# thuml/HashGAN

Hardware: AMD Instinct MI355X
Metric: queries/sec (mAP@R of Q queries vs N-code database, Hamming ranking) (higher is better)
Workload: dtype fp4 (E2M1 0/+-1) x fp4 -> f32 exact distances; u32 xor+popcount elsewhere; f64 AP; 1 GPU; C2: Q=10000 N=1000000 b=64 R=5000 C=10, planted codes; parallelism=1 GPU

## Files before the change

hashgan_amd/csrc/hg_core.hip:

```cpp
#include "hg_ctx.hpp"
#include "hg_host_pack.hpp"

#include <exception>
#include <map>
#include <mutex>
#include <thread>
#include <unistd.h>

thread_local std::string g_err;

int fail(int code, const char* fmt, ...) {
    char buf[512];
    va_list ap;
    va_start(ap, fmt);
    vsnprintf(buf, sizeof buf, fmt, ap);
    va_end(ap);
    g_err = buf;
    return code;
}

const char* const kKernelNames[KI_COUNT] = {"k_hist", "k_hist_reduce", "k_plan", "k_seg_counts", "k_seg_layout", "k_guess",
                                            "k_select", "k_rank_hist", "k_order", "k_rank_fused", "k_match", "k_ap", "k_merge", "k_pack",
                                            "k_real_sample", "k_real_guess", "k_real_select", "k_radix_pass", "k_real_finish", "k_select_mx", "k_rank_cnt", "rccl_allgather", "step_gpu_span", "k_real_rescore",
                                            "k_hist_rel", "k_hist_rel_reduce", "k_graded", "k_grade_hist", "k_grade_hist_reduce", "k_tie_ap"};
// ... 305 lines not shown
                    int64_t idx_base, int64_t n_total) {
    if (!c) return fail(HG_ERR_ARG, "hg_set_database: null context");
    if (N < 1 || !codes || !labels) return fail(HG_ERR_ARG, "hg_set_database: need N >= 1 and data");
    if (b < 1 || b > HG_MAX_BITS) return fail(HG_ERR_ARG, "hg_set_database: b=%d outside 1..%d", b, HG_MAX_BITS);
    if (C < 1) return fail(HG_ERR_ARG, "hg_set_database: C=%d", C);
    if (idx_base < 0 || n_total < N || idx_base + N > n_total || n_total >= 0xFFFFFFFFll)
        return fail(HG_ERR_ARG, "hg_set_database: shard [%lld, %lld) does not fit a database of %lld rows (< 2^32 - 1)",
                    (long long)idx_base, (long long)(idx_base + N), (long long)n_total);
    HG_TRY(c->use());
    c->N = N; c->b = b; c->C = C; c->n_total = n_total;
    c->NW = (b + 31) / 32; c->NB = b + 1; c->LW = (C + 63) / 64;
    c->idx_base = (u32)idx_base;
    c->bpad = 0;
    c->dbf_resident = false;
    HG_TRY(upload_codes(c, c->db, codes, N, (b + 63) / 64, c->NW));
    HG_TRY(c->dblab.reserve((size_t)(N > 0 ? N : 1) * c->LW * 8));
    if (N) HG_HIP(hipMemcpyAsync(c->dblab.p, labels, (size_t)N * c->LW * 8, hipMemcpyHostToDevice, c->stream));
    HG_TRY(c->sync());
    c->stage = ST_DB;
    c->dbx_valid = false;
    c->dbx3_valid = false;
    c->dbx4_valid = false;
    c->dbx8_valid = false;
    c->bet_consecutive_fail = c->shard_bet_fail = 0;
    c->cap_boost = c->real_cap_boost = 1;
    c->crowd_probed = false;
    c->cfg_epoch++;
    c->db_gen++;
    return HG_OK;
}

static int pack_on_device(hg_ctx* c, const float* x, const int64_t* lab, i64 n, DevBuf& codes, DevBuf& labels,
                          DevBuf& feats, int64_t* bad_codes, int64_t* bad_labels, i64 (&census)[3]) {
    const int b = c->b, C = c->C, NW = c->NW, LW = c->LW;
    const int bpad = (b + 15) / 16 * 16;
    c->bpad = bpad;
    const size_t fb = (size_t)n * bpad * 4, lb = (size_t)n * C * 8;
    HG_TRY(feats.reserve(fb + 256));
    HG_TRY(c->stage_in.reserve(lb));
    HG_TRY(c->badcnt.reserve(32));
    HG_TRY(codes.reserve((size_t)n * NW * 4 + 64 * 4));
    HG_TRY(labels.reserve((size_t)n * LW * 8));
    HG_HIP(hipMemsetAsync(c->badcnt.p, 0, 32, c->stream));
    if (bpad != b) HG_HIP(hipMemsetAsync(feats.p, 0, fb, c->stream));
    HG_HIP(hipMemcpy2DAsync(feats.p, (size_t)bpad * 4, x, (size_t)b * 4, (size_t)b * 4, (size_t)n, hipMemcpyHostToDevice, c->stream));
    c->t_begin(KI_PACK);
// ... 153 lines not shown
    if (N < 1 || !host_x || !host_labels) return fail(HG_ERR_ARG, "hg_set_database_f32: need N >= 1 and data");
    if (b < 1 || b > HG_MAX_BITS) return fail(HG_ERR_ARG, "hg_set_database_f32: b=%d outside 1..%d", b, HG_MAX_BITS);
    if (C < 1) return fail(HG_ERR_ARG, "hg_set_database_f32: C=%d", C);
    if (idx_base < 0 || n_total < N || idx_base + N > n_total || n_total >= 0xFFFFFFFFll)
        return fail(HG_ERR_ARG, "hg_set_database_f32: shard [%lld, %lld) does not fit a database of %lld rows (< 2^32 - 1)",
                    (long long)idx_base, (long long)(idx_base + N), (long long)n_total);
    HG_TRY(c->use());
    c->N = N; c->b = b; c->C = C; c->n_total = n_total;
    c->NW = (b + 31) / 32; c->NB = b + 1; c->LW = (C + 63) / 64;
    c->idx_base = (u32)idx_base;
    if (c->opt.host_pack) {
        HG_TRY(pack_on_host(c, host_x, host_labels, N, c->db, c->dblab, c->dbf, (int)c->opt.keep_floats, &c->dbf_resident,
                            bad_codes, bad_labels, c->census_db));
    } else {
        HG_TRY(pack_on_device(c, host_x, host_labels, N, c->db, c->dblab, c->dbf, bad_codes, bad_labels, c->census_db));
        c->dbf_resident = true;
    }
    if (!c->dbf_resident) c->bpad = 0;
    c->stage = ST_DB;
    c->dbx_valid = false;
    c->dbx3_valid = false;
    c->dbx4_valid = false;
    c->dbx8_valid = false;
    c->dbfx_valid = false;
    c->dbfb_valid = false;
    c->bet_consecutive_fail = c->shard_bet_fail = 0;
    c->cap_boost = c->real_cap_boost = 1;
    c->crowd_probed = false;
    c->cfg_epoch++;
    c->db_gen++;
    return HG_OK;
}

static __global__ __launch_bounds__(256) void k_copy_in(const u32* __restrict__ src_a, u32* __restrict__ dst_a, const i64 na, const int sw, const int dw,
                                                        const u32* __restrict__ src_b, u32* __restrict__ dst_b, const i64 nb) {
    const i64 i = (i64)blockIdx.x * 256 + threadIdx.x;
    if (i < na) { const i64 r = i / dw; dst_a[i] = src_a[r * sw + (i - r * dw)]; }
    else if (i - na < nb) dst_b[i - na] = src_b[i - na];
}

static void queries_replaced(hg_ctx* c, i64 old_q, bool had_q) {
    const bool carry = had_q && old_q == c->Q && c->map_warm_R >= 0 && c->map_warm_cfg == c->cfg_epoch;
    c->cfg_epoch++;
    c->q_gen++;
    if (carry) c->map_warm_cfg = c->cfg_epoch;
}

int hg_set_queries_f32(hg_ctx* c, const float* host_x, const int64_t* host_labels, int64_t Q, int64_t* bad_codes,
                       int64_t* bad_labels) {
    HG_TRY(need(c, ST_DB, "hg_set_queries_f32", "hg_set_database"));
    if (Q < 1 || !host_x || !host_labels) return fail(HG_ERR_ARG, "hg_set_queries_f32: need Q >= 1 and data");
    if (Q > 0x7FFFFFC0ll) return fail(HG_ERR_ARG, "hg_set_queries_f32: Q too large");
    const i64 old_q = c->Q;
    const bool had_q = (c->stage & ST_Q) != 0;
    c->Q = Q;
    if (c->opt.host_pack) {
        const int saved_bpad = c->bpad;
        HG_TRY(pack_on_host(c, host_x, host_labels, Q, c->qc, c->qlab, c->qf, c->dbf_resident ? 1 : 0, &c->qf_resident,
                            bad_codes, bad_labels, c->census_q));
        if (!c->qf_resident) c->bpad = saved_bpad;
    } else {
        HG_TRY(pack_on_device(c, host_x, host_labels, Q, c->qc, c->qlab, c->qf, bad_codes, bad_labels, c->census_q));
        c->qf_resident = true;
    }
    c->stage = ST_DB | ST_Q;
    c->qx_valid = false;
    queries_replaced(c, old_q, had_q);
    return HG_OK;
}

int hg_get_packed(hg_ctx* c, int which, uint32_t* host_codes, uint64_t* host_labels) {
    HG_TRY(need(c, which ? (ST_DB | ST_Q) : ST_DB, "hg_get_packed", "hg_set_database / hg_set_queries"));
    const i64 n = which ? c->Q : c->N;
    DevBuf& cd = which ? c->qc : c->db;
    DevBuf& lb = which ? c->qlab : c->dblab;
    if (host_codes) HG_HIP(hipMemcpyAsync(host_codes, cd.p, (size_t)n * c->NW * 4, hipMemcpyDeviceToHost, c->stream));
    if (host_labels) HG_HIP(hipMemcpyAsync(host_labels, lb.p, (size_t)n * c->LW * 8, hipMemcpyDeviceToHost, c->stream));
    return c->sync();
}

int hg_set_queries(hg_ctx* c, const uint64_t* codes, const uint64_t* labels, int64_t Q) {
    HG_TRY(need(c, ST_DB, "hg_set_queries", "hg_set_database"));
    if (Q < 1 || !codes || !labels) return fail(HG_ERR_ARG, "hg_set_queries: need Q >= 1 and data");
    if (Q > 0x7FFFFFC0ll) return fail(HG_ERR_ARG, "hg_set_queries: Q too large");
    const i64 old_q = c->Q;
    const bool had_q = (c->stage & ST_Q) != 0;
    c->Q = Q;
    const int W = (c->b + 63) / 64;
    const size_t cb = (size_t)Q * W * 8, lb = (size_t)Q * c->LW * 8;
// ... 3 lines not shown
    if (qs.cap < cb + lb) {
        pin_free(qs.pin, qs.cap);
        qs.pin = nullptr; qs.cap = 0;
        HG_HIP(pin_alloc(&qs.pin, cb + lb, &qs.cap));
    }
    if (!qs.ev) HG_HIP(hipEventCreateWithFlags(&qs.ev, hipEventDisableTiming));
    memcpy(qs.pin, codes, cb);
    memcpy((char*)qs.pin + cb, labels, lb);
    HG_TRY(c->qc.reserve((size_t)Q * c->NW * 4 + 64 * 4));
    HG_TRY(c->qlab.reserve(lb));
    if (cb + lb <= ((size_t)4 << 20)) {
        const i64 nc = (i64)Q * c->NW, nl = (i64)Q * c->LW * 2;
        hipLaunchKernelGGL(k_copy_in, dim3(grid_for(nc + nl)), dim3(256), 0, c->stream, (const u32*)qs.pin, c->qc.as<u32>(), nc, 2 * W, c->NW,
                           (const u32*)((const char*)qs.pin + cb), c->qlab.as<u32>(), nl);
        HG_TRY(c->check_launch("k_copy_in"));
    } else {
        HG_TRY(upload_codes(c, c->qc, (const uint64_t*)qs.pin, Q, W, c->NW));
        HG_HIP(hipMemcpyAsync(c->qlab.p, (const char*)qs.pin + cb, lb, hipMemcpyHostToDevice, c->stream));
    }
    HG_HIP(hipEventRecord(qs.ev, c->stream));
    qs.used = true;
    c->stage = ST_DB | ST_Q;
    c->qx_valid = false;
    c->qf_resident = false;
    queries_replaced(c, old_q, had_q);
    return HG_OK;
}

extern "C++" int do_match(hg_ctx* c) {
    const Geo& g = c->geo;
    const i64 nKB = (g.R + 255) / 256;
    const i64 blocks = nKB * g.Q;
    if (blocks > 0x7FFFFFFFll) return fail(HG_ERR_ARG, "hg_match: Q*R too large for one launch");
    c->t_begin(KI_MATCH);
    hipLaunchKernelGGL(k_match, dim3((unsigned)blocks), dim3(256), 0, c->stream, c->out_idx.as<u32>(),
                       c->dblab.as<u64>(), c->qlab.as<u64>(), c->mbits.as<u64>(), c->RW, (int)nKB, g);
    c->t_end();
    HG_TRY(c->check_launch("k_match"));
    c->stage |= ST_MATCH;
    c->stage &= ~(unsigned)ST_AP;
    return HG_OK;
}

int hg_match(hg_ctx* c) {
    HG_TRY(need(c, ST_SELECT, "hg_match", "hg_select"));
    if (c->stage & ST_MATCH) return HG_OK;
// ... 264 lines not shown
        c->own_stream = true;
    }
    if (c->sub) c->sub->stream = c->stream;
    return HG_OK;
}

namespace {
struct OptionKey { const char* key; i64 Options::*field; bool flag; i64 lo, hi; const char* range; };
constexpr i64 kMax = INT64_MAX;
constexpr OptionKey flag(const char* k, i64 Options::*f) { return {k, f, true, 0, 1, nullptr}; }
constexpr OptionKey ranged(const char* k, i64 Options::*f, i64 lo, i64 hi, const char* range) { return {k, f, false, lo, hi, range}; }
const OptionKey kOptionKeys[] = {
    ranged("target_units", &Options::target_units, 1, kMax, "target_units must be >= 1"),
    ranged("min_segment", &Options::min_segment, 16, kMax, "min_segment must be >= 16"),
    ranged("max_segments", &Options::max_segments, 1, kMax, "max_segments must be >= 1"),
    ranged("sample_stride", &Options::sample_stride, 0, 1024, "sample_stride must be 0 (auto) .. 1024"),
    ranged("guess_sigma", &Options::guess_sigma, 0, 64, "guess_sigma must be 0..64"),
    ranged("cand_budget_x10", &Options::cand_budget_x10, 11, 1000, "cand_budget_x10 must be 11..1000"),
    flag("second_bet", &Options::second_bet),
    flag("crowd_probe", &Options::crowd_probe),
    flag("select_mfma", &Options::select_mfma),
    ranged("select_packed", &Options::select_packed, INT64_MIN, kMax, nullptr),
    flag("compact_records", &Options::compact_records),
    ranged("hist_mfma", &Options::hist_mfma, 0, 2, "hist_mfma must be 0, 1 or 2"),
    ranged("rank_lds", &Options::rank_lds, 0, 2, "rank_lds must be 0, 1 or 2"),
    ranged("rank_slices", &Options::rank_slices, 0, kMax, "rank_slices must be >= 0 (the smallest R it takes; 0: off)"),
    ranged("rank_dense", &Options::rank_dense, 0, 2, "rank_dense must be 0 or 1 (2 is accepted and means 1)"),
    ranged("rank_dense_gbm", &Options::rank_dense_gbm, -1, 1, "rank_dense_gbm must be -1, 0 or 1"),
    ranged("dense_budget_mb", &Options::dense_budget_mb, 1, kMax, "dense_budget_mb must be >= 1"),
    flag("all_rows_shortcut", &Options::all_rows_shortcut),
    flag("fuse_ap", &Options::fuse_ap),
    flag("inline_leftovers", &Options::inline_leftovers),
    flag("ap_wide", &Options::ap_wide),
    flag("ap_recip", &Options::ap_recip),
#if HG_PROBES
    ranged("probe_select", &Options::probe_select, INT64_MIN, kMax, nullptr),
#endif
    flag("stage_sync", &Options::stage_sync),
    flag("defer_verdict", &Options::defer_verdict),
    flag("staged_lists", &Options::staged_lists),
    flag("step_graph", &Options::step_graph),
    ranged("step_streams", &Options::step_streams, 1, 2, "step_streams must be 1 or 2"),
    ranged("timing_every", &Options::timing_every, 1, 1024, "timing_every must be 1..1024"),
    flag("host_pack", &Options::host_pack),
    ranged("keep_floats", &Options::keep_floats, 0, 2, "keep_floats must be 0, 1 or 2"),
    ranged("real_mfma", &Options::real_mfma, 0, 2, "real_mfma must be 0, 1 or 2"),
// ... 101 lines not shown
        const char* rest = key + 5;
        int kind = -1;
        if (!strncmp(rest, "us_", 3)) { kind = 0; rest += 3; }
        else if (!strncmp(rest, "n_", 2)) { kind = 1; rest += 2; }
        else if (!strncmp(rest, "max_us_", 7)) { kind = 2; rest += 7; }
        int ph = -1;
        for (int i = 0; i < HP_COUNT; ++i) if (!strcmp(rest, kHostPhaseNames[i])) ph = i;
        if (kind < 0 || ph < 0) return fail(HG_ERR_ARG, "hg_get_stat: unknown key '%s'", key);
        *value = kind == 0 ? g_host_ns[ph].load() / 1000 : kind == 1 ? g_host_calls[ph].load() : g_host_max_ns[ph].load() / 1000;
    }
    else if (!strcmp(key, "graph_replays")) *value = c->graph_replays;
    else if (!strcmp(key, "cut_beyond_planes")) {
        u32 v = 0;
        if (c->beyond.p) {
            HG_HIP(hipMemcpyAsync(&v, c->beyond.p, 4, hipMemcpyDeviceToHost, c->stream));
            HG_TRY(c->sync());
        }
        *value = v;
    }
    else if (!strcmp(key, "map_async_steps")) *value = c->map_async_steps;
    else if (!strcmp(key, "map_async_redone")) *value = c->map_async_redone;
    else if (!strcmp(key, "map_overlapped_steps")) *value = c->map_overlapped;
    else if (!strcmp(key, "segments")) *value = c->geo.S;
    else if (!strcmp(key, "records_kept")) {
        const Geo& g = c->geo;
        *value = -1;
        if (c->optimistic && c->sl_cnt.p && c->sl_cnt.cap >= (size_t)g.S * g.Qpad * 4) {
            HG_TRY(c->use());
            HG_TRY(c->sync());
            std::vector<u32> h((size_t)g.S * g.Qpad);
            HG_HIP(hipMemcpy(h.data(), c->sl_cnt.p, h.size() * 4, hipMemcpyDeviceToHost));
            i64 total = 0;
            for (int s = 0; s < g.S; ++s) for (int q = 0; q < g.Q; ++q) total += h[(size_t)s * g.Qpad + q];
            *value = total;
        }
    }
    else return fail(HG_ERR_ARG, "hg_get_stat: unknown key '%s'", key);
    return HG_OK;
}

int hg_get_census(hg_ctx* c, int queries, int64_t out[4]) {
    if (!c || !out) return fail(HG_ERR_ARG, "hg_get_census: null argument");
    const i64* cs = queries ? c->census_q : c->census_db;
    out[0] = cs[0]; out[1] = cs[1]; out[2] = cs[2];
    out[3] = (queries ? c->qf_resident : c->dbf_resident) ? 1 : 0;
    return HG_OK;
// ... 37 lines not shown
```

hashgan_amd/csrc/hg_ctx.hpp:

```cpp
#pragma once
#include "hg_kernels.hpp"
#pragma GCC visibility push(default)
#include "../../include/hashgan_amd.h"
#pragma GCC visibility pop

#include <rccl/rccl.h>
#include <atomic>
#include <chrono>
#include <cmath>
#include <cstdarg>
#include <cstdio>
#include <cstdlib>
#include <cstring>
#include <string>
#include <utility>
#include <vector>

using namespace hg;

extern thread_local std::string g_err;
int fail(int code, const char* fmt, ...);

#define HG_HIP(expr)                                                                         \
    do {                                                                                     \
// ... 150 lines not shown
                KI_ORDER, KI_RANK_FUSED, KI_MATCH, KI_AP, KI_MERGE, KI_PACK, KI_REAL_SAMPLE, KI_REAL_GUESS, KI_REAL_SELECT,
                KI_RADIX, KI_REAL_FINISH, KI_SELECT_MX, KI_RANK_LDS, KI_COMM, KI_STEP, KI_REAL_RESCORE, KI_HIST_REL, KI_HIST_REL_REDUCE,
                KI_GRADED, KI_GRADE_HIST, KI_GRADE_HIST_REDUCE, KI_TIE_AP, KI_COUNT };
enum Stage { ST_NONE = 0, ST_DB = 1, ST_Q = 2, ST_HIST = 4, ST_PLAN = 8, ST_SELECT = 16, ST_MATCH = 32, ST_AP = 64 };
extern const char* const kKernelNames[KI_COUNT];

void build_shape(int n, ApShape& sh);

struct Pending { int id; hipEvent_t a, b; };

struct Options {
    i64 target_units = 16384;
    i64 min_segment = 256;
    i64 max_segments = 2048;
    i64 optimistic = 1;
    i64 sample_stride = 0;
    i64 guess_sigma = 5;
    i64 cand_budget_x10 = 40;
    i64 second_bet = 1;
    i64 crowd_probe = 1;
    i64 select_mfma = 1;
    i64 select_packed = 3;
    i64 compact_records = 1;
    i64 hist_mfma = 2;
    i64 rank_lds = 2;
    i64 rank_slices = 7000;
    i64 rank_dense = 1;
    i64 rank_dense_gbm = -1;
    i64 dense_budget_mb = 16384;
    i64 all_rows_shortcut = 1;
    i64 fuse_ap = 1;
    i64 inline_leftovers = 1;
    i64 ap_wide = 1;
    i64 ap_recip = 1;
    i64 probe_select = 0;
    i64 stage_sync = 1;
    i64 defer_verdict = 0;
    i64 staged_lists = 1;
    i64 step_graph = 0;
    i64 step_streams = 2;
    i64 timing_every = 1;
    i64 host_pack = 1;
    i64 keep_floats = 2;
    i64 real_mfma = 2;
    i64 real_sample_half = 1;
    i64 real_second_sample = 1;
// ... 74 lines not shown
    Options opt;

    i64 N = 0, Q = 0, R = 0, n_total = 0;
    int b = 0, C = 0, NW = 0, NB = 0, LW = 0;
    u32 idx_base = 0;
    int G = 1, rank = 0;

    bool crowd_probed = false;
    i64 crowd_x100 = 0;
    i64 cap_boost = 1;
    i64 real_cap_boost = 1;
    bool leftovers_expected = false;
    bool last_leftovers_inline = false;

    bool want_lists = true;
    i64 bet_runs = 0, bet_fallbacks = 0, bet_requeried = 0;
    i64 rank_leftovers = 0;
    int bet_consecutive_fail = 0;
    int shard_bet_fail = 0;
    hg_ctx* sub = nullptr;
    bool is_sub = false;

    bool dbx_valid = false, qx_valid = false, dbx8_valid = false, dbx3_valid = false, dbx4_valid = false;
    bool hist_pairs = false;
    i64 bet_rebets = 0;
    bool rh_done = false;
    unsigned long long rh_q_gen = 0, rh_db_gen = 0;
    i64 rh_Q = 0, rh_Qpad = 0, rh_NB = 0;
    int last_rel_hist = 0;
    bool gr_done = false, gr_kept = false;
    unsigned long long gr_q_gen = 0, gr_db_gen = 0;
    i64 gr_Q = 0, gr_R = 0;
    int gr_nk = 0;
    bool gh_done = false;
    unsigned long long gh_q_gen = 0, gh_db_gen = 0;
    i64 gh_Q = 0, gh_Qpad = 0, gh_G = 0;
    bool ta_done = false;
    unsigned long long ta_q_gen = 0, ta_db_gen = 0;
    i64 ta_Q = 0;
    int ta_nR = 0;
    bool verdict_pending = false, verdict_known = false;
    int verdict_flag = 0;
    void* pin = nullptr;
    size_t pin_cap = 0;
    struct MapSlot {
        void* pin = nullptr; size_t cap = 0; hipEvent_t ev = nullptr;
// ... 29 lines not shown
    i64 real_requeried = 0;
    int bpad = 0;
    i64 census_db[3] = {0, 0, 0}, census_q[3] = {0, 0, 0};
    hipStream_t stream2 = nullptr;
    hipEvent_t stream2_ev = nullptr;
    size_t fstage_cap = 0;
    void* fstage = nullptr;
    hipEvent_t fstage_ev[4] = {nullptr, nullptr, nullptr, nullptr};
    void* hpk = nullptr;
    size_t hpk_cap = 0;
    bool dbf_resident = false, qf_resident = false;
    RealState real;
    bool real_lists = false;
    i64 shapes_for_R = -1;
    i64 recip_for_R = -1;

    ncclComm_t comm = nullptr;
    int comm_rank = 0, comm_world = 1;

    DevBuf db, dblab, qc, qlab;
    DevBuf dbf, qf;
    DevBuf dbx, qx;
    DevBuf dbx8;
    DevBuf rh_part, rh_all, rh_rel;
    DevBuf gr_tab, gr_out, gr_grades;
    DevBuf gh_part, gh_tab;
    DevBuf ta_tab, ta_out;
    DevBuf dbx3;
    DevBuf dbx4;
    DevBuf dbfx;
    DevBuf dbfb, xmax2;
    DevBuf shapes, ap_recip;
    DevBuf seglt, segtie;
    DevBuf mbits2;
    DevBuf part;
    DevBuf obuf[2];
    DevBuf beyond;
    DevBuf stage_in, badcnt;
    DevBuf flist;
    DevBuf dbytes;
    DevBuf samp, thr, sortA, sortB, scores, gtab;
    DevBuf sampx;
    DevBuf cntq;
    DevBuf krows;
    DevBuf thr2;
    DevBuf hist2;
    DevBuf gathered[4], scratch[4], comm_tmp, gath_idx, gath_dist;

    template <class F> void for_each_buf(F&& f) {
        for (DevBuf* d : {&db, &dblab, &qc, &qlab, &dbf, &qf}) f(*d, BUF_TABLE);
        for (DevBuf* d : {&dbx, &qx, &dbx8, &dbx3, &dbx4, &dbfx, &dbfb, &xmax2, &shapes, &ap_recip}) f(*d, BUF_DERIVED);
        for (DevBuf* d : {&seglt, &segtie, &mbits2, &part, &obuf[0], &obuf[1], &beyond, &stage_in, &badcnt, &flist, &dbytes, &samp, &thr,
                          &sortA, &sortB, &scores, &gtab, &sampx, &cntq, &krows, &thr2, &hist2, &comm_tmp, &gath_idx, &gath_dist, &rh_part, &rh_all, &rh_rel,
                          &gr_tab, &gr_out, &gr_grades, &gh_part, &gh_tab, &ta_tab, &ta_out})
            f(*d, BUF_WORK);
        for (DevBuf& d : gathered) f(d, BUF_WORK);
        for (DevBuf& d : scratch) f(d, BUF_WORK);
        for_each_step_buf(f);
        ws_b.for_each_step_buf(f);
    }
    void forget_derived() {
        dbx_valid = qx_valid = dbx8_valid = dbx3_valid = dbx4_valid = dbfx_valid = dbfb_valid = false;
        rh_done = false;
        gr_done = gr_kept = gh_done = ta_done = false;
        shapes_for_R = recip_for_R = -1;
        outblk_q = ws_b.outblk_q = -1;
    }

    struct StepGraph {
        hipGraph_t graph = nullptr;
        hipGraphExec_t exec = nullptr;
        unsigned long long epoch = 0, cfg = 0, seen_epoch = 0, seen_cfg = 0;
        i64 R = -1, seen_R = -1;
        int timing = -1, seen_timing = -1;
        StepState left;
        std::vector<Pending> evs;
    } sg;
    unsigned long long cfg_epoch = 1;
    bool capturing = false;
    i64 graph_replays = 0, graph_captures = 0;

    int timing = 0;
    double t_ms[KI_COUNT] = {0};
    i64 t_n[KI_COUNT] = {0};
    std::vector<Pending> pending;
// ... 89 lines not shown
inline int grid_for(i64 n, int per_block = 256) { return (int)((n + per_block - 1) / per_block); }
inline int padded_grid(int nBlk) { return (nBlk + 7) / 8 * 8; }

int need(hg_ctx* c, unsigned st, const char* who, const char* what);
int upload_codes(hg_ctx* c, DevBuf& dst, const uint64_t* host, i64 n, int W, int NW);
int ensure_pin(hg_ctx* c, size_t need_b);
int do_match(hg_ctx* c);
int ensure_ap_tables(hg_ctx* c, bool* use_recip);
int do_ap_range(hg_ctx* c, i64 q0, i64 nq, const u32* only = nullptr);
inline int do_ap(hg_ctx* c) { return do_ap_range(c, 0, c->geo.Q); }
int ensure_out_block(hg_ctx* c);
int read_plan_flag(hg_ctx* c, int* flag);
int launch_min_topr(hg_ctx* c, const u32* idx_all, const u8* dist_all, i64 n, int G);
hg_ctx* requery_child(hg_ctx* c, i64 nF);
int stage_ap_download(hg_ctx* c, void* dst = nullptr);
int wait_verdict(hg_ctx* c, bool staged, int* flag);
void make_geometry(hg_ctx* c);
Geo hist_geometry(const hg_ctx* c);
int set_R(hg_ctx* c, int64_t R, int G, int rank);
int launch_hist(hg_ctx* c);
int launch_hist_rel(hg_ctx* c, const Geo& g);
int launch_select_valu(hg_ctx* c, int lw, bool optimistic);
int launch_select_dense(hg_ctx* c, int lw);
int ensure_mx_images(hg_ctx* c, bool need_db);
int launch_hist_mx(hg_ctx* c);
int launch_select_mx(hg_ctx* c, int lw, const int* cut);
int launch_select_mx3(hg_ctx* c, int lw, const int* cut);
int launch_select_mx4(hg_ctx* c, int lw, const int* cut);
int preload_valu(); int preload_mx(); int preload_mx1(); int preload_real(); int preload_seq();
void comm_release(hg_ctx* c);

#define HG_DISPATCH_NW(fn, c, ...)                              \
    switch ((c)->NW) {                                          \
        case 1: return fn<1>(c, ##__VA_ARGS__);                 \
        case 2: return fn<2>(c, ##__VA_ARGS__);                 \
        case 3: return fn<3>(c, ##__VA_ARGS__);                 \
        case 4: return fn<4>(c, ##__VA_ARGS__);                 \
        case 5: return fn<5>(c, ##__VA_ARGS__);                 \
        case 6: return fn<6>(c, ##__VA_ARGS__);                 \
        case 7: return fn<7>(c, ##__VA_ARGS__);                 \
        case 8: return fn<8>(c, ##__VA_ARGS__);                 \
        default: return fail(HG_ERR_ARG, "unsupported code length: %d words", (c)->NW); \
    }
```

hashgan_amd/csrc/hg_hist_i8.hpp:

```cpp
#pragma once
#include "hg_kernels.hpp"
#include "hg_hist_mx.hpp"

namespace hg {

typedef int i32x16 __attribute__((ext_vector_type(16)));
typedef __attribute__((address_space(3))) u32 lds_u32;

__device__ __forceinline__ void lds_add_at(const u32 addr, const u32 inc) {
#if defined(__HIP_DEVICE_COMPILE__)
    __hip_atomic_fetch_add((lds_u32*)addr, inc, __ATOMIC_RELAXED, __HIP_MEMORY_SCOPE_WORKGROUP);
#else
    (void)addr; (void)inc;
#endif
}

__device__ __forceinline__ uint4 bits16_to_bytes(const u32 bits, const u32 one, const u32 zero) {
    u32 w[4];
#pragma unroll
    for (int d = 0; d < 4; ++d) {
        u32 v = 0;
#pragma unroll
        for (int i = 0; i < 4; ++i) v |= (((bits >> (4 * d + i)) & 1u) ? one : zero) << (8 * i);
        w[d] = v;
    }
    return uint4{w[0], w[1], w[2], w[3]};
}

static __global__ __launch_bounds__(256) void k_expand_db_i8(const u32* __restrict__ db, uint4* __restrict__ img, i64 N, i64 n16, int NW) {
    const i64 i = (i64)blockIdx.x * 256 + threadIdx.x;
    if (i >= n16 * NW * 2) return;
    const i64 row = i / (NW * 2);
    const int c = (int)(i - row * NW * 2), m = c >> 1, hh = c & 1;
    const u32 word = row < N ? db[row * NW + m] : 0u;
    img[(((row >> 4) * NW + m) * 2 + hh) * 16 + (row & 15)] = bits16_to_bytes((word >> (16 * hh)) & 0xFFFFu, 8u, 0u);
}

constexpr int hist_i8_cols(bool pack16) { return pack16 ? 1 : 2; }

template <int NW, bool PACK16>
__global__ __launch_bounds__(256) __attribute__((amdgpu_waves_per_eu(4, 4)))
void k_hist_i8(const u32* __restrict__ qc, const u8* __restrict__ dbx8, u32* __restrict__ hist, const Geo g) {
    extern __shared__ __attribute__((aligned(16))) u32 hlds[];
    constexpr int QT = 2, WQ = 32 * QT;
    const int lb = logical_block(g.nBlk);
    if (lb < 0) return;
    const int lane = threadIdx.x & 63;
    const int wave = __builtin_amdgcn_readfirstlane(threadIdx.x >> 6);
    const int nQB = g.nQT;
    const int sp = lb / nQB, qb = lb - sp * nQB;
    const int h = lane >> 5, j = lane & 31;
    const int NB = g.NB, b = g.NB - 1;
    const i64 lo0 = (i64)(2 * sp) * g.L, lo1 = lo0 + g.L;
    const i64 len0 = (lo0 + g.L < g.N ? g.L : g.N - lo0);
    const i64 len1 = lo1 >= g.N ? 0 : (lo1 + g.L < g.N ? g.L : g.N - lo1);
    const i64 mylen = h ? len1 : len0;
    const i64 ntile = ((len0 > len1 ? len0 : len1) + 15) / 16;
    const i64 NG = (g.N + 15) >> 4;
    const int stride = g.hist_stride;

    constexpr int NCOL = hist_i8_cols(PACK16);
    u32* col = hlds + wave * NCOL * NB * 32;
    for (int i = lane; i < NCOL * NB * 32; i += 64) col[i] = 0u;

    const int q0w = (qb * WPB + wave) * WQ;
    i32x4 bq[QT][NW];
    i32x16 biasv[QT];
    u32 inc[QT];
#pragma unroll
    for (int t = 0; t < QT; ++t) {
        const int q = q0w + t * 32 + j;
        int pop = 0;
#pragma unroll
        for (int m = 0; m < NW; ++m) {
            const u32 word = q < g.Q ? qc[(i64)q * NW + m] : 0u;
            pop += __builtin_popcount(word);
            const int first = 32 * m + 16 * h;
            const u32 valid = b - first >= 16 ? 0xFFFFu : (b - first <= 0 ? 0u : (1u << (b - first)) - 1u);
            const u32 bits = (word >> (16 * h)) & 0xFFFFu;
            const uint4 neg = bits16_to_bytes(bits & valid, 0xF0u, 0u);
            const uint4 pos = bits16_to_bytes(~bits & valid, 0x10u, 0u);
            bq[t][m] = i32x4{(int)(neg.x | pos.x), (int)(neg.y | pos.y), (int)(neg.z | pos.z), (int)(neg.w | pos.w)};
        }
        u32* c0 = col + (PACK16 ? 0 : t * NB * 32) + j;
        const int base = (int)(u32)(size_t)(lds_u32*)c0 + 128 * pop;
#pragma unroll
        for (int r = 0; r < 16; ++r) biasv[t][r] = base;
        inc[t] = PACK16 ? (t ? 65536u : 1u) : 1u;
    }
    wave_lds_sync();

    const int ah = (j >> 2) & 1;
    const int ar = (j & 3) + 4 * (j >> 3);
    const i64 ag0 = (ah ? lo1 : lo0) >> 4;
    auto chunk = [&](const i64 T, const int m) -> i32x4 {
        i64 G = ag0 + T;
        G = G < NG ? G : NG - 1;
        return *(const i32x4*)(dbx8 + ((((G * NW + m) * 2 + h) * 16 + ar) * 16));
    };
    i32x4 av[NW];
    if (ntile > 0) {
#pragma unroll
        for (int m = 0; m < NW; ++m) av[m] = chunk(0, m);
    }
    for (i64 T = 0; T < ntile; T += stride) {
        i32x4 an[NW];
        const i64 Tn = T + stride < ntile ? T + stride : T;
#pragma unroll
        for (int m = 0; m < NW; ++m) an[m] = chunk(Tn, m);
        const i64 left = mylen - T * 16;
        const bool whole = __all(left >= 16);
#pragma unroll
        for (int t = 0; t < QT; ++t) {
            i32x16 acc = biasv[t];
#pragma unroll
            for (int m = 0; m < NW; ++m) acc = __builtin_amdgcn_mfma_i32_32x32x32_i8(av[m], bq[t][m], acc, 0, 0, 0);
            if (whole) {
#pragma unroll
                for (int r = 0; r < 16; ++r)
                    lds_add_at((u32)acc[r], inc[t]);
            } else {
#pragma unroll
                for (int r = 0; r < 16; ++r)
                    if ((i64)r < left) lds_add_at((u32)acc[r], inc[t]);
            }
        }
#pragma unroll
        for (int m = 0; m < NW; ++m) av[m] = an[m];
    }
    wave_lds_sync();
    const int q = q0w + lane;
    if (q < g.Qpad) {
        u32* __restrict__ out = hist + (i64)sp * NB * g.Qpad + q;
        const int dn = g.hcap > 0 && g.hcap < NB ? g.hcap : NB;
        for (int d = 0; d < dn; ++d) {
            const u32 v = PACK16 ? (col[d * 32 + j] >> (16 * h)) & 0xFFFFu : col[(h * NB + d) * 32 + j];
            out[(i64)d * g.Qpad] = v;
        }
    }
}

}
```

hashgan_amd/csrc/hg_pairs_mx.hip:

```cpp
#include "hg_ctx.hpp"
#include "hg_mx_drain.hpp"
#include "hg_select_mx.hpp"
#include "hg_select_mx3.hpp"
#include "hg_select_mx4.hpp"
#include "hg_hist_mx.hpp"
#include "hg_hist_i8.hpp"

int ensure_mx_images(hg_ctx* c, const bool need_db) {
    const int NW = c->NW, NM = (NW + 1) / 2;
    if (need_db && !c->dbx_valid) {
        const i64 n16 = (c->N + 15) / 16 * 16;
        HG_TRY(c->dbx.reserve((size_t)(n16 > 0 ? n16 : 16) * NM * 32));
        const i64 items = n16 * 2 * NM;
        c->t_begin(KI_PACK);
        if (items) hipLaunchKernelGGL(k_expand_db, dim3(grid_for(items)), dim3(256), 0, c->stream, c->db.as<u32>(),
                                      c->dbx.as<uint4>(), (i64)c->N, n16, NW, NM);
        c->t_end();
        HG_TRY(c->check_launch("k_expand_db"));
        c->dbx_valid = true;
    }
    if (!c->qx_valid) {
        const i64 qpad = ((i64)c->Q + 511) / 512 * 512;
        HG_TRY(c->qx.reserve((size_t)qpad * NM * 32));
        const i64 items = qpad * 2 * NM;
        c->t_begin(KI_PACK);
        hipLaunchKernelGGL(k_expand_queries, dim3(grid_for(items)), dim3(256), 0, c->stream, c->qc.as<u32>(), c->qx.as<uint4>(),
                           (i64)c->Q, qpad, NW, NM);
        c->t_end();
        HG_TRY(c->check_launch("k_expand_queries"));
        c->qx_valid = true;
    }
    return HG_OK;
}


namespace {
template <int NW> int launch_hist_mx_t(hg_ctx* c) {
    HG_TRY(ensure_mx_images(c, true));
    Geo g = c->geo;
    const int nSP = (g.S + 1) / 2;
    const int nQB = (g.Q + 255) / 256;
    g.nQT = nQB;
    g.nUnits = (i64)nSP * nQB;
    g.wpb = WPB;
    g.nBlk = (int)g.nUnits;
    const i64 tiles_per_half = ((g.L + 15) / 16 + g.hist_stride - 1) / g.hist_stride;
    const i64 visited_per_pair = 2 * tiles_per_half * 16;
    const bool pack16 = visited_per_pair < 65536;
    const size_t lds = (size_t)WPB * (pack16 ? 1 : 2) * g.NB * 32 * 4;
    c->t_begin(KI_HIST);
    if (pack16) {
        hipLaunchKernelGGL((k_hist_mx<NW, true>), dim3(padded_grid(g.nBlk)), dim3(256), lds, c->stream, c->qc.as<u32>(), c->qx.as<u8>(),
                           c->dbx.as<u8>(), c->hist.as<u32>(), g);
// ... 27 lines not shown
    g.nQT = nQB;
    g.nUnits = (i64)nSP * nQB;
    g.wpb = P::WPB;
    g.nBlk = (int)g.nUnits;
    const PackedLds L = packed_lds_layout<P>(NW, LW);
    if (L.total > 64 * 1024)
        HG_HIP(hipFuncSetAttribute(reinterpret_cast<const void*>(kernel), hipFuncAttributeMaxDynamicSharedMemorySize, L.total));
    SelArgs a{cut, c->sl_start.as<u32>(), c->sl_tie.as<u32>(), c->sl_cnt.as<u32>(),
              c->failq.as<u32>(), c->cap, c->crow, 1, c->sstar.as<int>(), (int)c->opt.probe_select};
    c->t_begin(KI_SELECT_MX);
    hipLaunchKernelGGL(kernel, dim3(padded_grid(g.nBlk)), dim3(64 * P::WPB), (size_t)L.total, c->stream, c->qc.as<u32>(),
                       c->qlab.as<u64>(), c->qx.as<u8>(), c->db.as<u32>(), image.as<u8>(), c->dblab.as<u64>(), a,
                       c->cand.as<u8>(), g);
    c->t_end();
    return c->check_launch(kernel_name);
}
template <int NW, int LW> int launch_select_mx3_t(hg_ctx* c, const int* cut) {
    return launch_select_packed<M3Pack>(c, cut, NW, LW, c->dbx3, c->dbx3_valid, k_expand_db3, "k_expand_db3", &k_select_mx3<NW, LW>, "k_select_mx3");
}
template <int NW, int LW> int launch_select_mx4_t(hg_ctx* c, const int* cut) {
    return launch_select_packed<M4Pack>(c, cut, NW, LW, c->dbx4, c->dbx4_valid, k_expand_db4, "k_expand_db4", &k_select_mx4<NW, LW>, "k_select_mx4");
}

template <int NW> int launch_hist_i8_t(hg_ctx* c) {
    if (!c->dbx8_valid) {
        const i64 n16 = (c->N + 15) / 16 * 16;
        HG_TRY(c->dbx8.reserve((size_t)n16 * NW * 32));
        c->t_begin(KI_PACK);
        hipLaunchKernelGGL(k_expand_db_i8, dim3(grid_for(n16 * NW * 2)), dim3(256), 0, c->stream, c->db.as<u32>(), c->dbx8.as<uint4>(),
                           (i64)c->N, n16, NW);
        c->t_end();
        HG_TRY(c->check_launch("k_expand_db_i8"));
        c->dbx8_valid = true;
    }
    Geo g = c->geo;
    const int nSP = (g.S + 1) / 2;
    const int nQB = (g.Q + 255) / 256;
    g.nQT = nQB;
    g.nUnits = (i64)nSP * nQB;
    g.wpb = WPB;
    g.nBlk = (int)g.nUnits;
    const i64 tiles_per_half = ((g.L + 15) / 16 + g.hist_stride - 1) / g.hist_stride;
    const bool pack16 = 2 * tiles_per_half * 16 < 65536;
    const size_t lds = (size_t)WPB * hist_i8_cols(pack16) * g.NB * 32 * 4;
    c->t_begin(KI_HIST);
    if (pack16) {
        if (lds > 64 * 1024)
            HG_HIP(hipFuncSetAttribute(reinterpret_cast<const void*>(&k_hist_i8<NW, true>), hipFuncAttributeMaxDynamicSharedMemorySize, (int)lds));
        hipLaunchKernelGGL((k_hist_i8<NW, true>), dim3(padded_grid(g.nBlk)), dim3(256), lds, c->stream, c->qc.as<u32>(), c->dbx8.as<u8>(),
                           c->hist.as<u32>(), g);
    } else {
        if (lds > 64 * 1024)
            HG_HIP(hipFuncSetAttribute(reinterpret_cast<const void*>(&k_hist_i8<NW, false>), hipFuncAttributeMaxDynamicSharedMemorySize, (int)lds));
        hipLaunchKernelGGL((k_hist_i8<NW, false>), dim3(padded_grid(g.nBlk)), dim3(256), lds, c->stream, c->qc.as<u32>(), c->dbx8.as<u8>(),
                           c->hist.as<u32>(), g);
    }
    c->t_end();
    return c->check_launch("k_hist_i8");
}
}

int launch_hist_mx(hg_ctx* c) {
    if (c->opt.hist_mfma == 2 && c->NW <= 4) {
        switch (c->NW) {
            case 1: return launch_hist_i8_t<1>(c);
            case 2: return launch_hist_i8_t<2>(c);
            case 3: return launch_hist_i8_t<3>(c);
            default: return launch_hist_i8_t<4>(c);
        }
    }
    HG_DISPATCH_NW(launch_hist_mx_t, c)
}


int launch_select_mx4(hg_ctx* c, int lw, const int* cut) {
    if (c->NW < 3 || c->NW > 4 || lw < 1 || lw > 2) return fail(HG_ERR_ARG, "k_select_mx4 takes codes of 65..128 bits and 1..128 classes");
    if (c->NW == 3) return lw == 1 ? launch_select_mx4_t<3, 1>(c, cut) : launch_select_mx4_t<3, 2>(c, cut);
    return lw == 1 ? launch_select_mx4_t<4, 1>(c, cut) : launch_select_mx4_t<4, 2>(c, cut);
}

int launch_select_mx3(hg_ctx* c, int lw, const int* cut) {
// ... 11 lines not shown
```

hashgan_amd/csrc/hg_seq.hip:

```cpp
#include "hg_ctx.hpp"
#include <chrono>
#include "hg_select_mx.hpp"
#include "hg_select_mx3.hpp"
#include "hg_select_mx4.hpp"
#include "hg_hist_mx.hpp"
#include "hg_hist_rel.hpp"
#include "hg_graded.hpp"
#include "hg_tie_ap.hpp"
#include "hg_rank_cnt.hpp"
#include "hg_rank_lean.hpp"
#include "hg_rank_dense.hpp"

constexpr i64 SAMPLE_RATIO = 2;

void make_geometry(hg_ctx* c) {
    Geo& g = c->geo;
    g.Q = (int)c->Q;
    g.nQT = (int)((c->Q + 63) / 64);
    g.Qpad = g.nQT * 64;
    g.NW = c->NW; g.NB = c->NB; g.LW = c->LW;
    g.N = c->N; g.R = c->R; g.idx_base = c->idx_base;
    i64 S = (c->opt.target_units + g.nQT - 1) / g.nQT;
    if (S > c->opt.max_segments) S = c->opt.max_segments;
    const i64 maxS = (c->N + c->opt.min_segment - 1) / c->opt.min_segment;
// ... 1482 lines not shown

int hg_topr(hg_ctx* c, int64_t R) {
    HG_TRY(need(c, ST_DB | ST_Q, "hg_topr", "hg_set_database + hg_set_queries"));
    return run_oneshot(c, R, true, false);
}

int hg_map(hg_ctx* c, int64_t R, double* host_ap, int64_t* host_rel) {
    HG_TRY(need(c, ST_DB | ST_Q, "hg_map", "hg_set_database + hg_set_queries"));
    const i64 fails0 = c->bet_fallbacks + c->bet_requeried + c->bet_rebets, left0 = c->rank_leftovers;
    c->last_leftovers_inline = false;
    HG_TRY(run_oneshot(c, R, false, true));
    HG_TRY(hg_get_ap(c, host_ap, host_rel));
    if (c->optimistic && c->bet_fallbacks + c->bet_requeried + c->bet_rebets == fails0 && (c->rank_leftovers == left0 || c->last_leftovers_inline) && !c->is_sub) {
        c->map_warm_cfg = c->cfg_epoch; c->map_warm_epoch = g_alloc_epoch; c->map_warm_R = R;
        if (c->opt.step_streams >= 2 && c->own_stream && !c->stream_b) HG_TRY(stream_create(c->device, &c->stream_b));
    } else {
        c->map_warm_R = -1;
    }
    return HG_OK;
}

static int prepare_shared(hg_ctx* c, int64_t R, bool* enqueued) {
    *enqueued = false;
    if (c->opt.select_mfma && !c->qx_valid) { HG_TRY(ensure_mx_images(c, false)); *enqueued = true; }
    const bool recip = c->opt.ap_recip && R <= (1ll << 20);
    if (c->shapes_for_R != R || (recip && c->recip_for_R != R)) {
        HG_TRY(set_R(c, R, 1, 0));
        bool use_recip = false;
        HG_TRY(ensure_ap_tables(c, &use_recip));
        *enqueued = true;
    }
    return HG_OK;
}

static int enqueue_bet_on_b(hg_ctx* c, hg_ctx::MapSlot& m, int64_t R, int stride, bool tail_fork) {
    if (!c->stream_b) HG_TRY(stream_create(c->device, &c->stream_b));
    if (!c->ev_pre) HG_HIP(hipEventCreateWithFlags(&c->ev_pre, hipEventDisableTiming));
    if (!c->ev_fork) HG_HIP(hipEventCreateWithFlags(&c->ev_fork, hipEventDisableTiming));
    if (tail_fork || !c->pre_valid) {
        HG_HIP(hipEventRecord(c->ev_fork, c->stream));
        HG_HIP(hipStreamWaitEvent(c->stream_b, c->ev_fork, 0));
    } else {
        HG_HIP(hipStreamWaitEvent(c->stream_b, c->ev_pre, 0));
    }
    c->b_open = false;
    const unsigned long long e0 = g_alloc_epoch.load();
    c->swap_step();
// ... 105 lines not shown
```

Baseline: 12.53 million queries/s.

## Precompute int8 query images and run hist kernel as persistent blocks

Adds a separate kernel that expands query codes into int8 MFMA operand images plus popcounts once and caches them, so the histogram kernel loads them instead of rebuilding them per block. The histogram kernel becomes persistent: the grid is sized from occupancy times CU count, and each block walks a contiguous run of (query block, segment) units. It reloads query operands only when the query block changes and drains LDS counters with atomic exchange so they can be reused. This cuts the per-block query expansion and launch cost, in exchange for an extra image buffer, an extra pre-pass kernel and serial per-block work that may balance less evenly.

```diff
diff --git a/hashgan_amd/csrc/hg_core.hip b/hashgan_amd/csrc/hg_core.hip
--- a/hashgan_amd/csrc/hg_core.hip
+++ b/hashgan_amd/csrc/hg_core.hip
@@ -351,6 +351,7 @@
     c->dbx3_valid = false;
     c->dbx4_valid = false;
     c->dbx8_valid = false;
+    c->qx8_valid = false;
     c->bet_consecutive_fail = c->shard_bet_fail = 0;
     c->cap_boost = c->real_cap_boost = 1;
     c->crowd_probed = false;
@@ -550,6 +551,7 @@
     c->dbx3_valid = false;
     c->dbx4_valid = false;
     c->dbx8_valid = false;
+    c->qx8_valid = false;
     c->dbfx_valid = false;
     c->dbfb_valid = false;
     c->bet_consecutive_fail = c->shard_bet_fail = 0;
@@ -593,6 +595,7 @@
     }
     c->stage = ST_DB | ST_Q;
     c->qx_valid = false;
+    c->qx8_valid = false;
     queries_replaced(c, old_q, had_q);
     return HG_OK;
 }
@@ -642,6 +645,7 @@
     qs.used = true;
     c->stage = ST_DB | ST_Q;
     c->qx_valid = false;
+    c->qx8_valid = false;
     c->qf_resident = false;
     queries_replaced(c, old_q, had_q);
     return HG_OK;
@@ -952,6 +956,7 @@
     flag("select_mfma", &Options::select_mfma),
     ranged("select_packed", &Options::select_packed, INT64_MIN, kMax, nullptr),
     flag("compact_records", &Options::compact_records),
+    ranged("hist_blocks", &Options::hist_blocks, 0, 1 << 20, "hist_blocks must be 0 (auto) .. 1048576"),
     ranged("hist_mfma", &Options::hist_mfma, 0, 2, "hist_mfma must be 0, 1 or 2"),
     ranged("rank_lds", &Options::rank_lds, 0, 2, "rank_lds must be 0, 1 or 2"),
     ranged("rank_slices", &Options::rank_slices, 0, kMax, "rank_slices must be >= 0 (the smallest R it takes; 0: off)"),
@@ -1099,6 +1104,9 @@
     else if (!strcmp(key, "map_async_redone")) *value = c->map_async_redone;
     else if (!strcmp(key, "map_overlapped_steps")) *value = c->map_overlapped;
     else if (!strcmp(key, "segments")) *value = c->geo.S;
+    else if (!strcmp(key, "segment_rows")) *value = c->geo.L;
+    else if (!strcmp(key, "hist_stride")) *value = c->geo.hist_stride;
+    else if (!strcmp(key, "hist_blocks_used")) *value = c->hist_blocks_used;
     else if (!strcmp(key, "records_kept")) {
         const Geo& g = c->geo;
         *value = -1;
diff --git a/hashgan_amd/csrc/hg_ctx.hpp b/hashgan_amd/csrc/hg_ctx.hpp
--- a/hashgan_amd/csrc/hg_ctx.hpp
+++ b/hashgan_amd/csrc/hg_ctx.hpp
@@ -196,6 +196,7 @@
     i64 select_mfma = 1;
     i64 select_packed = 3;
     i64 compact_records = 1;
+    i64 hist_blocks = 0;
     i64 hist_mfma = 2;
     i64 rank_lds = 2;
     i64 rank_slices = 7000;
@@ -316,6 +317,10 @@
     bool is_sub = false;
 
     bool dbx_valid = false, qx_valid = false, dbx8_valid = false, dbx3_valid = false, dbx4_valid = false;
+    bool qx8_valid = false;
+    i64 hist_occ_key = -1;
+    int hist_occ = 0;
+    i64 hist_blocks_used = 0;
     bool hist_pairs = false;
     i64 bet_rebets = 0;
     bool rh_done = false;
@@ -391,6 +396,7 @@
     DevBuf dbf, qf;
     DevBuf dbx, qx;
     DevBuf dbx8;
+    DevBuf qx8;
     DevBuf rh_part, rh_all, rh_rel;
     DevBuf gr_tab, gr_out, gr_grades;
     DevBuf gh_part, gh_tab;
@@ -418,7 +424,7 @@
 
     template <class F> void for_each_buf(F&& f) {
         for (DevBuf* d : {&db, &dblab, &qc, &qlab, &dbf, &qf}) f(*d, BUF_TABLE);
-        for (DevBuf* d : {&dbx, &qx, &dbx8, &dbx3, &dbx4, &dbfx, &dbfb, &xmax2, &shapes, &ap_recip}) f(*d, BUF_DERIVED);
+        for (DevBuf* d : {&dbx, &qx, &dbx8, &qx8, &dbx3, &dbx4, &dbfx, &dbfb, &xmax2, &shapes, &ap_recip}) f(*d, BUF_DERIVED);
         for (DevBuf* d : {&seglt, &segtie, &mbits2, &part, &obuf[0], &obuf[1], &beyond, &stage_in, &badcnt, &flist, &dbytes, &samp, &thr,
                           &sortA, &sortB, &scores, &gtab, &sampx, &cntq, &krows, &thr2, &hist2, &comm_tmp, &gath_idx, &gath_dist, &rh_part, &rh_all, &rh_rel,
                           &gr_tab, &gr_out, &gr_grades, &gh_part, &gh_tab, &ta_tab, &ta_out})
@@ -429,7 +435,7 @@
         ws_b.for_each_step_buf(f);
     }
     void forget_derived() {
-        dbx_valid = qx_valid = dbx8_valid = dbx3_valid = dbx4_valid = dbfx_valid = dbfb_valid = false;
+        dbx_valid = qx_valid = qx8_valid = dbx8_valid = dbx3_valid = dbx4_valid = dbfx_valid = dbfb_valid = false;
         rh_done = false;
         gr_done = gr_kept = gh_done = ta_done = false;
         shapes_for_R = recip_for_R = -1;
@@ -565,7 +571,7 @@
 int launch_hist_rel(hg_ctx* c, const Geo& g);
 int launch_select_valu(hg_ctx* c, int lw, bool optimistic);
 int launch_select_dense(hg_ctx* c, int lw);
-int ensure_mx_images(hg_ctx* c, bool need_db);
+int ensure_mx_images(hg_ctx* c, bool need_db, bool need_q8 = false);
 int launch_hist_mx(hg_ctx* c);
 int launch_select_mx(hg_ctx* c, int lw, const int* cut);
 int launch_select_mx3(hg_ctx* c, int lw, const int* cut);
diff --git a/hashgan_amd/csrc/hg_hist_i8.hpp b/hashgan_amd/csrc/hg_hist_i8.hpp
--- a/hashgan_amd/csrc/hg_hist_i8.hpp
+++ b/hashgan_amd/csrc/hg_hist_i8.hpp
@@ -36,107 +36,141 @@
     img[(((row >> 4) * NW + m) * 2 + hh) * 16 + (row & 15)] = bits16_to_bytes((word >> (16 * hh)) & 0xFFFFu, 8u, 0u);
 }
 
+static __global__ __launch_bounds__(256) void k_expand_queries_i8(const u32* __restrict__ qc, uint4* __restrict__ img, int* __restrict__ pop,
+                                                                  i64 Q, i64 qpad, int NW, int b) {
+    const i64 i = (i64)blockIdx.x * 256 + threadIdx.x;
+    if (i >= qpad * NW * 2) return;
+    const int lane = (int)(i & 63), h = lane >> 5, j = lane & 31;
+    const i64 c = i >> 6, tile = c / NW;
+    const int m = (int)(c - tile * NW);
+    const i64 q = tile * 32 + j;
+    const u32 word = q < Q ? qc[q * NW + m] : 0u;
+    const int first = 32 * m + 16 * h;
+    const u32 valid = b - first >= 16 ? 0xFFFFu : (b - first <= 0 ? 0u : (1u << (b - first)) - 1u);
+    const u32 bits = (word >> (16 * h)) & 0xFFFFu;
+    const uint4 neg = bits16_to_bytes(bits & valid, 0xF0u, 0u);
+    const uint4 pos = bits16_to_bytes(~bits & valid, 0x10u, 0u);
+    img[i] = uint4{neg.x | pos.x, neg.y | pos.y, neg.z | pos.z, neg.w | pos.w};
+    if (m == 0 && h == 0) {
+        int p = 0;
+        for (int w = 0; w < NW; ++w) p += __builtin_popcount(q < Q ? qc[q * NW + w] : 0u);
+        pop[q] = p;
+    }
+}
+inline size_t hist_i8_qimage_bytes(i64 qpad, int NW) { return (size_t)qpad * NW * 32; }
+
 constexpr int hist_i8_cols(bool pack16) { return pack16 ? 1 : 2; }
 
 template <int NW, bool PACK16>
 __global__ __launch_bounds__(256) __attribute__((amdgpu_waves_per_eu(4, 4)))
-void k_hist_i8(const u32* __restrict__ qc, const u8* __restrict__ dbx8, u32* __restrict__ hist, const Geo g) {
+void k_hist_i8(const u8* __restrict__ qx8, const int* __restrict__ qpop, const u8* __restrict__ dbx8, u32* __restrict__ hist, const Geo g,
+               const int nSP, const int run, const int rem) {
     extern __shared__ __attribute__((aligned(16))) u32 hlds[];
     constexpr int QT = 2, WQ = 32 * QT;
     const int lb = logical_block(g.nBlk);
     if (lb < 0) return;
     const int lane = threadIdx.x & 63;
     const int wave = __builtin_amdgcn_readfirstlane(threadIdx.x >> 6);
-    const int nQB = g.nQT;
-    const int sp = lb / nQB, qb = lb - sp * nQB;
     const int h = lane >> 5, j = lane & 31;
-    const int NB = g.NB, b = g.NB - 1;
-    const i64 lo0 = (i64)(2 * sp) * g.L, lo1 = lo0 + g.L;
-    const i64 len0 = (lo0 + g.L < g.N ? g.L : g.N - lo0);
-    const i64 len1 = lo1 >= g.N ? 0 : (lo1 + g.L < g.N ? g.L : g.N - lo1);
-    const i64 mylen = h ? len1 : len0;
-    const i64 ntile = ((len0 > len1 ? len0 : len1) + 15) / 16;
+    const int NB = g.NB;
     const i64 NG = (g.N + 15) >> 4;
     const int stride = g.hist_stride;
+    const int dn = g.hcap > 0 && g.hcap < NB ? g.hcap : NB;
+    const int u0 = lb * run + (lb < rem ? lb : rem), nu = run + (lb < rem ? 1 : 0);
+    int qb = u0 / nSP, sp = u0 - qb * nSP;
 
     constexpr int NCOL = hist_i8_cols(PACK16);
     u32* col = hlds + wave * NCOL * NB * 32;
     for (int i = lane; i < NCOL * NB * 32; i += 64) col[i] = 0u;
-
-    const int q0w = (qb * WPB + wave) * WQ;
-    i32x4 bq[QT][NW];
-    i32x16 biasv[QT];
-    u32 inc[QT];
-#pragma unroll
-    for (int t = 0; t < QT; ++t) {
-        const int q = q0w + t * 32 + j;
-        int pop = 0;
-#pragma unroll
-        for (int m = 0; m < NW; ++m) {
-            const u32 word = q < g.Q ? qc[(i64)q * NW + m] : 0u;
-            pop += __builtin_popcount(word);
-            const int first = 32 * m + 16 * h;
-            const u32 valid = b - first >= 16 ? 0xFFFFu : (b - first <= 0 ? 0u : (1u << (b - first)) - 1u);
-            const u32 bits = (word >> (16 * h)) & 0xFFFFu;
-            const uint4 neg = bits16_to_bytes(bits & valid, 0xF0u, 0u);
-            const uint4 pos = bits16_to_bytes(~bits & valid, 0x10u, 0u);
-            bq[t][m] = i32x4{(int)(neg.x | pos.x), (int)(neg.y | pos.y), (int)(neg.z | pos.z), (int)(neg.w | pos.w)};
-        }
-        u32* c0 = col + (PACK16 ? 0 : t * NB * 32) + j;
-        const int base = (int)(u32)(size_t)(lds_u32*)c0 + 128 * pop;
-#pragma unroll
-        for (int r = 0; r < 16; ++r) biasv[t][r] = base;
-        inc[t] = PACK16 ? (t ? 65536u : 1u) : 1u;
-    }
     wave_lds_sync();
 
     const int ah = (j >> 2) & 1;
     const int ar = (j & 3) + 4 * (j >> 3);
-    const i64 ag0 = (ah ? lo1 : lo0) >> 4;
-    auto chunk = [&](const i64 T, const int m) -> i32x4 {
-        i64 G = ag0 + T;
-        G = G < NG ? G : NG - 1;
-        return *(const i32x4*)(dbx8 + ((((G * NW + m) * 2 + h) * 16 + ar) * 16));
-    };
-    i32x4 av[NW];
-    if (ntile > 0) {
+    i32x4 bq[QT][NW];
+    int base[QT] = {0, 0};
+    int cur = -1;
+    for (int u = 0; u < nu; ++u) {
+        const int q0w = (qb * WPB + wave) * WQ;
+        if (q0w < g.Qpad) {
+            if (qb != cur) {
+                cur = qb;
 #pragma unroll
-        for (int m = 0; m < NW; ++m) av[m] = chunk(0, m);
-    }
-    for (i64 T = 0; T < ntile; T += stride) {
-        i32x4 an[NW];
-        const i64 Tn = T + stride < ntile ? T + stride : T;
+                for (int t = 0; t < QT; ++t) {
+                    const i64 tile = (i64)(q0w >> 5) + t;
 #pragma unroll
-        for (int m = 0; m < NW; ++m) an[m] = chunk(Tn, m);
-        const i64 left = mylen - T * 16;
-        const bool whole = __all(left >= 16);
+                    for (int m = 0; m < NW; ++m) bq[t][m] = *(const i32x4*)(qx8 + ((tile * NW + m) * 64 + lane) * 16);
+                    u32* c0 = col + (PACK16 ? 0 : t * NB * 32) + j;
+                    base[t] = (int)(u32)(size_t)(lds_u32*)c0 + 128 * qpop[q0w + t * 32 + j];
+                }
+            }
+            i32x16 biasv[QT];
 #pragma unroll
-        for (int t = 0; t < QT; ++t) {
-            i32x16 acc = biasv[t];
+            for (int t = 0; t < QT; ++t)
 #pragma unroll
-            for (int m = 0; m < NW; ++m) acc = __builtin_amdgcn_mfma_i32_32x32x32_i8(av[m], bq[t][m], acc, 0, 0, 0);
-            if (whole) {
+                for (int r = 0; r < 16; ++r) biasv[t][r] = base[t];
+            const i64 lo0 = (i64)(2 * sp) * g.L, lo1 = lo0 + g.L;
+            const i64 len0 = (lo0 + g.L < g.N ? g.L : g.N - lo0);
+            const i64 len1 = lo1 >= g.N ? 0 : (lo1 + g.L < g.N ? g.L : g.N - lo1);
+            const i64 mylen = h ? len1 : len0;
+            const i64 ntile = ((len0 > len1 ? len0 : len1) + 15) / 16;
+            const i64 ag0 = (ah ? lo1 : lo0) >> 4;
+            auto chunk = [&](const i64 T, const int m) -> i32x4 {
+                i64 G = ag0 + T;
+                G = G < NG ? G : NG - 1;
+                return *(const i32x4*)(dbx8 + ((((G * NW + m) * 2 + h) * 16 + ar) * 16));
+            };
+            i32x4 av[NW];
 #pragma unroll
-                for (int r = 0; r < 16; ++r)
-                    lds_add_at((u32)acc[r], inc[t]);
+            for (int m = 0; m < NW; ++m) av[m] = chunk(0, m);
+            for (i64 T = 0; T < ntile; T += stride) {
+                i32x4 an[NW];
+                const i64 Tn = T + stride < ntile ? T + stride : T;
+#pragma unroll
+                for (int m = 0; m < NW; ++m) an[m] = chunk(Tn, m);
+                const i64 left = mylen - T * 16;
+                const bool whole = __all(left >= 16);
+#pragma unroll
+                for (int t = 0; t < QT; ++t) {
+                    i32x16 acc = biasv[t];
+#pragma unroll
+                    for (int m = 0; m < NW; ++m) acc = __builtin_amdgcn_mfma_i32_32x32x32_i8(av[m], bq[t][m], acc, 0, 0, 0);
+                    const u32 inc = PACK16 && t ? 65536u : 1u;
+                    if (whole) {
+#pragma unroll
+                        for (int r = 0; r < 16; ++r)
+                            lds_add_at((u32)acc[r], inc);
+                    } else {
+#pragma unroll
+                        for (int r = 0; r < 16; ++r)
+                            if ((i64)r < left) lds_add_at((u32)acc[r], inc);
+                    }
+                }
+#pragma unroll
+                for (int m = 0; m < NW; ++m) av[m] = an[m];
+            }
+            wave_lds_sync();
+            int ol = lane;
+            __asm__ volatile("" : "+v"(ol));
+            const int oh = ol >> 5, oj = ol & 31;
+            if (PACK16) {
+                u32* __restrict__ out = hist + ((i64)sp * NB + oh) * g.Qpad + q0w + oj;
+                u32* c = col + ol;
+                for (int d = oh; d < dn; d += 2, c += 64, out += 2 * (i64)g.Qpad) {
+                    const u32 v = __hip_atomic_exchange(c, 0u, __ATOMIC_RELAXED, __HIP_MEMORY_SCOPE_WORKGROUP);
+                    out[0] = v & 0xFFFFu;
+                    out[32] = v >> 16;
+                }
             } else {
-#pragma unroll
-                for (int r = 0; r < 16; ++r)
-                    if ((i64)r < left) lds_add_at((u32)acc[r], inc[t]);
+                u32* __restrict__ out = hist + (i64)sp * NB * g.Qpad + q0w + ol;
+                u32* c = col + oh * NB * 32 + oj;
+                for (int d = 0; d < dn; ++d, c += 32, out += g.Qpad) {
+                    const u32 v = __hip_atomic_exchange(c, 0u, __ATOMIC_RELAXED, __HIP_MEMORY_SCOPE_WORKGROUP);
+                    out[0] = v;
+                }
             }
+            wave_lds_sync();
         }
-#pragma unroll
-        for (int m = 0; m < NW; ++m) av[m] = an[m];
-    }
-    wave_lds_sync();
-    const int q = q0w + lane;
-    if (q < g.Qpad) {
-        u32* __restrict__ out = hist + (i64)sp * NB * g.Qpad + q;
-        const int dn = g.hcap > 0 && g.hcap < NB ? g.hcap : NB;
-        for (int d = 0; d < dn; ++d) {
-            const u32 v = PACK16 ? (col[d * 32 + j] >> (16 * h)) & 0xFFFFu : col[(h * NB + d) * 32 + j];
-            out[(i64)d * g.Qpad] = v;
-        }
+        if (++sp == nSP) { sp = 0; ++qb; }
     }
 }
 
diff --git a/hashgan_amd/csrc/hg_pairs_mx.hip b/hashgan_amd/csrc/hg_pairs_mx.hip
--- a/hashgan_amd/csrc/hg_pairs_mx.hip
+++ b/hashgan_amd/csrc/hg_pairs_mx.hip
@@ -6,7 +6,7 @@
 #include "hg_hist_mx.hpp"
 #include "hg_hist_i8.hpp"
 
-int ensure_mx_images(hg_ctx* c, const bool need_db) {
+int ensure_mx_images(hg_ctx* c, const bool need_db, const bool need_q8) {
     const int NW = c->NW, NM = (NW + 1) / 2;
     if (need_db && !c->dbx_valid) {
         const i64 n16 = (c->N + 15) / 16 * 16;
@@ -29,6 +29,17 @@
         c->t_end();
         HG_TRY(c->check_launch("k_expand_queries"));
         c->qx_valid = true;
+    }
+    if (need_q8 && !c->qx8_valid) {
+        const i64 qpad = ((i64)c->Q + 255) / 256 * 256;
+        const size_t img = hist_i8_qimage_bytes(qpad, NW);
+        HG_TRY(c->qx8.reserve(img + (size_t)qpad * 4));
+        c->t_begin(KI_PACK);
+        hipLaunchKernelGGL(k_expand_queries_i8, dim3(grid_for(qpad * NW * 2)), dim3(256), 0, c->stream, c->qc.as<u32>(), c->qx8.as<uint4>(),
+                           (int*)(c->qx8.as<char>() + img), (i64)c->Q, qpad, NW, c->b);
+        c->t_end();
+        HG_TRY(c->check_launch("k_expand_queries_i8"));
+        c->qx8_valid = true;
     }
     return HG_OK;
 }
@@ -102,7 +113,29 @@
     return launch_select_packed<M4Pack>(c, cut, NW, LW, c->dbx4, c->dbx4_valid, k_expand_db4, "k_expand_db4", &k_select_mx4<NW, LW>, "k_select_mx4");
 }
 
+template <int NW, bool PACK16> int launch_hist_i8_p(hg_ctx* c, Geo g, const int nSP, const size_t lds) {
+    const void* fn = reinterpret_cast<const void*>(&k_hist_i8<NW, PACK16>);
+    if (lds > 64 * 1024) HG_HIP(hipFuncSetAttribute(fn, hipFuncAttributeMaxDynamicSharedMemorySize, (int)lds));
+    const i64 key = ((i64)lds << 4) | (NW << 1) | (PACK16 ? 1 : 0);
+    if (c->hist_occ_key != key) {
+        int per_cu = 0;
+        HG_HIP(hipOccupancyMaxActiveBlocksPerMultiprocessor(&per_cu, fn, 256, lds));
+        c->hist_occ = per_cu > 0 ? per_cu : 1;
+        c->hist_occ_key = key;
+    }
+    const i64 want = c->opt.hist_blocks > 0 ? c->opt.hist_blocks : (i64)c->n_cu * c->hist_occ;
+    g.nBlk = (int)(want < g.nUnits ? want : g.nUnits);
+    c->hist_blocks_used = g.nBlk;
+    const size_t img = hist_i8_qimage_bytes(((i64)c->Q + 255) / 256 * 256, NW);
+    c->t_begin(KI_HIST);
+    hipLaunchKernelGGL((k_hist_i8<NW, PACK16>), dim3(padded_grid(g.nBlk)), dim3(256), lds, c->stream, c->qx8.as<u8>(),
+                       (const int*)(c->qx8.as<char>() + img), c->dbx8.as<u8>(), c->hist.as<u32>(), g, nSP,
+                       (int)(g.nUnits / g.nBlk), (int)(g.nUnits % g.nBlk));
+    c->t_end();
+    return c->check_launch("k_hist_i8");
+}
 template <int NW> int launch_hist_i8_t(hg_ctx* c) {
+    HG_TRY(ensure_mx_images(c, false, true));
     if (!c->dbx8_valid) {
         const i64 n16 = (c->N + 15) / 16 * 16;
         HG_TRY(c->dbx8.reserve((size_t)n16 * NW * 32));
@@ -119,24 +152,10 @@
     g.nQT = nQB;
     g.nUnits = (i64)nSP * nQB;
     g.wpb = WPB;
-    g.nBlk = (int)g.nUnits;
     const i64 tiles_per_half = ((g.L + 15) / 16 + g.hist_stride - 1) / g.hist_stride;
     const bool pack16 = 2 * tiles_per_half * 16 < 65536;
     const size_t lds = (size_t)WPB * hist_i8_cols(pack16) * g.NB * 32 * 4;
-    c->t_begin(KI_HIST);
-    if (pack16) {
-        if (lds > 64 * 1024)
-            HG_HIP(hipFuncSetAttribute(reinterpret_cast<const void*>(&k_hist_i8<NW, true>), hipFuncAttributeMaxDynamicSharedMemorySize, (int)lds));
-        hipLaunchKernelGGL((k_hist_i8<NW, true>), dim3(padded_grid(g.nBlk)), dim3(256), lds, c->stream, c->qc.as<u32>(), c->dbx8.as<u8>(),
-                           c->hist.as<u32>(), g);
-    } else {
-        if (lds > 64 * 1024)
-            HG_HIP(hipFuncSetAttribute(reinterpret_cast<const void*>(&k_hist_i8<NW, false>), hipFuncAttributeMaxDynamicSharedMemorySize, (int)lds));
-        hipLaunchKernelGGL((k_hist_i8<NW, false>), dim3(padded_grid(g.nBlk)), dim3(256), lds, c->stream, c->qc.as<u32>(), c->dbx8.as<u8>(),
-                           c->hist.as<u32>(), g);
-    }
-    c->t_end();
-    return c->check_launch("k_hist_i8");
+    return pack16 ? launch_hist_i8_p<NW, true>(c, g, nSP, lds) : launch_hist_i8_p<NW, false>(c, g, nSP, lds);
 }
 }
 
diff --git a/hashgan_amd/csrc/hg_seq.hip b/hashgan_amd/csrc/hg_seq.hip
--- a/hashgan_amd/csrc/hg_seq.hip
+++ b/hashgan_amd/csrc/hg_seq.hip
@@ -1528,7 +1528,8 @@
 
 static int prepare_shared(hg_ctx* c, int64_t R, bool* enqueued) {
     *enqueued = false;
-    if (c->opt.select_mfma && !c->qx_valid) { HG_TRY(ensure_mx_images(c, false)); *enqueued = true; }
+    const bool q8 = c->opt.hist_mfma == 2 && c->NW <= 4;
+    if (c->opt.select_mfma && (!c->qx_valid || (q8 && !c->qx8_valid))) { HG_TRY(ensure_mx_images(c, false, q8)); *enqueued = true; }
     const bool recip = c->opt.ap_recip && R <= (1ll << 20);
     if (c->shapes_for_R != R || (recip && c->recip_for_R != R)) {
         HG_TRY(set_R(c, R, 1, 0));
```

Measured after the change: 12.50 million queries/s. About the same (-0.2%).
